# Oneaccount1/recommend-sys

Measured on NVIDIA B200. Metric: similarity_pairs_per_sec, higher is better.
Workload: dtype f64

## Files before the change

recommend-sys_b200/csrc/sim_stream.cu:

```cuda
#include <cstdlib>
#include <cstring>

#include "common.cuh"
#include "sim_terms.cuh"

namespace {

constexpr int SW = RS_STREAM_WARPS;

struct StreamArgs {
    const int64_t *l_ptr;
    const int32_t *l_col;
    const double *l_val;
    const int64_t *l2r;
    const int64_t *r_ptr;
    const int32_t *r_col;
    const double *r_dev;
    const int32_t *row_order;
    const int32_t *cp;
    int32_t n_chunks;
    const double *pmeans;
    const double *left_bias, *right_bias;
    double global_bias, shrinkage;
    double *sims;
    int64_t ld_s;
    int32_t n_left;
    int64_t row_begin, row_end;
    int64_t n_rows;
    int cyc_R;
    int symmetric;
    const int32_t *rank;
    const int32_t *lab_row;
    int32_t n_pop;
    unsigned long long *counter;
};

constexpr int G = 8;


struct PopArgs {
    const int32_t *rows;
    int64_t n_rows;
    const int32_t *rank;
    int32_t n_pop;
    const int32_t *pop_items;
    int32_t n_blk, ld;
    const void *dense;
    int64_t n_first;
    int32_t skip;
};

__device__ __forceinline__ void pop_cp_async16(void *dst, const void *src) {
    asm volatile("cp.async.cg.shared.global [%0], [%1], 16;" ::"r"((uint32_t)__cvta_generic_to_shared(dst)), "l"(src) : "memory");
}
__device__ __forceinline__ void pop_commit() { asm volatile("cp.async.commit_group;" ::: "memory"); }
template <int N> __device__ __forceinline__ void pop_wait() { asm volatile("cp.async.wait_group %0;" ::"n"(N) : "memory"); }

template <int SIM, bool SHRINK, typename DT>
__device__ __forceinline__ void pop_item(const StreamArgs &a, const PopArgs &pa, int64_t item, double *scratch, int lane) {
    constexpr bool U8 = sizeof(DT) == 1;
    double2 *s_a = reinterpret_cast<double2 *>(scratch);
    double *s_rbias = scratch + 64;
    int32_t *s_c = reinterpret_cast<int32_t *>(scratch + 96);
    uint8_t *s_d = reinterpret_cast<uint8_t *>(scratch + 112);
    const DT *__restrict__ dense = static_cast<const DT *>(pa.dense);
    const double nan_v = __longlong_as_double(0x7ff8000000000001ll);
    const int32_t i = pa.rows[item / pa.n_blk];
    const int b = (int)(item % pa.n_blk);
    const int pi = pa.rank[i] < pa.n_pop ? pa.rank[i] : -1;
    if (pi >= 0 && 32 * b > pi) return;
    const int col = 32 * b + lane;
    const int32_t hcol = pa.pop_items[col];
    const bool want = hcol >= 0 && (pi < 0 || col < pi);
    double bh = 0.0;
    if (want && SIM == RS_SIM_PEARSON) bh = a.pmeans[hcol];
    if (want && SIM == RS_SIM_PEARSON_BASELINE) bh = a.global_bias + a.left_bias[hcol];
    double ai = 0.0;
    if (SIM == RS_SIM_PEARSON) ai = a.pmeans[i];
    if (SIM == RS_SIM_PEARSON_BASELINE) ai = a.global_bias + a.left_bias[i];
    double acc0 = 0.0, acc1 = 0.0, acc2 = 0.0, acc3 = 0.0;
    const int64_t eb = a.l_ptr[i], ee = a.l_ptr[i + 1];

    auto apply = [&](bool rated, double rb, const double2 aa, double rbias_u) {
        (void)rbias_u;
        if (SIM == RS_SIM_MSD) {
            const double dd = aa.x - rb;
            const double t = dd * dd;
            if (rated) { acc0 += t; acc1 += 1.0; }
        } else {
            const double t1 = rb * rb, t2 = aa.x * rb;
            if (rated) {
                acc0 += aa.y;
                acc1 += t1;
                acc2 += t2;
                if (SHRINK) acc3 += 1.0;
            }
        }
    };

    if (__any_sync(0xffffffffu, want)) {
        int32_t c_0 = 0, c_1 = 0;
        double v_0 = 0.0, v_1 = 0.0;
        if (eb + lane < ee) { c_0 = a.l_col[eb + lane]; v_0 = a.l_val[eb + lane]; }
        if (eb + 32 + lane < ee) { c_1 = a.l_col[eb + 32 + lane]; v_1 = a.l_val[eb + 32 + lane]; }
        auto issue = [&](int32_t c_l, int64_t x0, int buf) {
            if constexpr (U8) {
#pragma unroll
                for (int h2 = 0; h2 < 2; h2++) {
                    const int p = lane + 32 * h2, u = p >> 1;
                    const int32_t c_u = __shfl_sync(0xffffffffu, c_l, u);
                    if (x0 + u < ee)
                        pop_cp_async16(s_d + buf * 1024 + 32 * u + 16 * (p & 1),
                                       reinterpret_cast<const uint8_t *>(dense) + (int64_t)c_u * pa.ld + 32 * b + 16 * (p & 1));
                }
            }
            pop_commit();
        };
        __syncwarp();
        issue(c_0, eb, 0);
        int buf = 0;
        for (int64_t x0 = eb; x0 < ee; x0 += 32, buf ^= 1) {
            const int32_t c = c_0;
            const double v = v_0;
            c_0 = c_1; v_0 = v_1;
            c_1 = 0; v_1 = 0.0;
            if (x0 + 64 + lane < ee) { c_1 = a.l_col[x0 + 64 + lane]; v_1 = a.l_val[x0 + 64 + lane]; }
            double ra = 0.0, rbias = 0.0;
            if (x0 + lane < ee) {
                if (SIM == RS_SIM_PEARSON) ra = v - ai;
                else if (SIM == RS_SIM_PEARSON_BASELINE) { rbias = a.right_bias[c]; const double bb = ai + rbias; ra = v - bb; }
                else ra = v;
            }
            s_a[lane] = make_double2(ra, ra * ra);
            if (SIM == RS_SIM_PEARSON_BASELINE) s_rbias[lane] = rbias;
            if (!U8) s_c[lane] = c;
            issue(c_0, x0 + 32, buf ^ 1);
            pop_wait<1>();
            __syncwarp();
            const int lim = (ee - x0) < 32 ? (int)(ee - x0) : 32;
            if constexpr (U8) {
                const uint8_t *sd = s_d + buf * 1024 + lane;
#pragma unroll 8
                for (int u = 0; u < lim; u++) {
                    const int code = want ? (int)sd[32 * u] : 0;
                    const double y = __hiloint2double(0x43380000, code) - (6755399441055744.0 + (double)RS_INT8_BIAS);
                    const double2 aa = s_a[u];
                    double rb;
                    double rbias_u = 0.0;
                    if (SIM == RS_SIM_PEARSON) rb = y - bh;
                    else if (SIM == RS_SIM_PEARSON_BASELINE) { rbias_u = s_rbias[u]; const double bb = bh + rbias_u; rb = y - bb; }
                    else rb = y;
                    apply(code != 0, rb, aa, rbias_u);
                }
            } else {
                constexpr int PU = 8;
                for (int u0 = 0; u0 < lim; u0 += PU) {
                    double d[PU];
#pragma unroll
                    for (int g = 0; g < PU; g++) {
                        d[g] = nan_v;
                        if (want && u0 + g < lim) d[g] = dense[(int64_t)s_c[u0 + g] * pa.ld + col];
                    }
#pragma unroll
                    for (int g = 0; g < PU; g++) {
                        const int u = (u0 + g) & 31;
                        apply(d[g] == d[g], d[g], s_a[u], 0.0);
                    }
                }
            }
            __syncwarp();
        }
        pop_wait<0>();
    }

    if (hcol >= 0) {
        double *out = a.sims + (a.cyc_R > 1 ? rs_cyc_local(i, a.cyc_R) : (int64_t)(i - a.row_begin)) * a.ld_s;
        if (pi >= 0 && col == pi) {
            out[hcol] = nan_v;
        } else if (want) {
            const double acc_r[4] = {acc0, acc1, acc2, acc3};
            out[hcol] = sim_value<SIM, SHRINK>(acc_r, 1, a.shrinkage);
        }
    }
}

template <int SIM, bool SHRINK, int SYM, int JC, int POP>
__global__ void __launch_bounds__(SW * 32, 4) sim_stream_kernel(StreamArgs a, PopArgs pa) {
    constexpr int NACC = SHRINK ? 4 : 3;
    extern __shared__ double s_acc_all[];
    const int warp = threadIdx.x >> 5, lane = threadIdx.x & 31;
    double *acc = s_acc_all + (size_t)warp * NACC * JC;
    double *s_ra = s_acc_all + (size_t)SW * NACC * JC + warp * 32;
    const int64_t Q = a.n_chunks;
    const int64_t n_items = a.n_rows * Q;
    const double nan_v = __longlong_as_double(0x7ff8000000000001ll);
    const int32_t *__restrict__ r_col = a.r_col;
    const double *__restrict__ r_dev = a.r_dev;

    for (;;) {
        unsigned long long item = 0;
        if (lane == 0) item = atomicAdd(a.counter, 1ull);
        item = __shfl_sync(0xffffffffu, item, 0);
        if (POP) {
            int64_t d = (int64_t)item;
            if (d >= pa.n_first) d = d >= pa.n_first + n_items ? d - n_items : -1;
            if (d >= pa.n_rows * pa.n_blk) break;
            if (pa.skip && ((d >= 0 && d < pa.n_first && (pa.skip & 1)) || (d < 0 && (pa.skip & 2)) || (d >= pa.n_first && (pa.skip & 4)))) continue;
            if (d >= 0) {
                __syncwarp();
                if (POP == 1) pop_item<SIM, SHRINK, uint8_t>(a, pa, d, acc, lane);
                else pop_item<SIM, SHRINK, double>(a, pa, d, acc, lane);
                __syncwarp();
                continue;
            }
            item -= (unsigned long long)pa.n_first;
        } else if ((int64_t)item >= n_items) break;
        const int64_t q = (int64_t)item % Q;
        const int32_t i = a.row_order[(int64_t)item / Q];
        const int32_t li = POP ? a.rank[i] - a.n_pop : i;
        const int j0 = (int)(q * JC);
        if (SYM == 1 && j0 + JC <= li) continue;
        if (SYM == 2 && j0 > li) continue;

        for (int x = lane; x < NACC * JC; x += 32) acc[x] = 0.0;

        double ai = 0.0;
        if (SIM == RS_SIM_PEARSON) ai = a.pmeans[i];
        if (SIM == RS_SIM_PEARSON_BASELINE) ai = a.global_bias + a.left_bias[i];

        const int64_t eb = a.l_ptr[i], ee = a.l_ptr[i + 1];
        for (int64_t x0 = eb; x0 < ee; x0 += 32) {
            const int64_t e = x0 + lane;
            double ra = 0.0;
            uint32_t lo = 0, self = 0xffffffffu;
            int n = 0;
            if (e < ee) {
                const int32_t c = a.l_col[e];
                const double v = a.l_val[e];
                if (SIM == RS_SIM_PEARSON) ra = v - ai;
                else if (SIM == RS_SIM_PEARSON_BASELINE) { const double bb = ai + a.right_bias[c]; ra = v - bb; }
                else ra = v;
                const int64_t rp = a.r_ptr[c];
                const int32_t *cpc = a.cp + (int64_t)c * (Q + 1) + q;
                int64_t lo64 = rp + cpc[0];
                int64_t hi = rp + cpc[1];
                const int64_t self64 = a.l2r[e];
                if (SYM == 1) { if (self64 + 1 > lo64) lo64 = self64 + 1; }
                else if (SYM == 2) { if (self64 < hi) hi = self64; }
                else self = (uint32_t)self64;
                n = hi > lo64 ? (int)(hi - lo64) : 0;
                lo = (uint32_t)lo64;
            }
            __syncwarp();
            s_ra[lane] = ra;
            __syncwarp();
            const int lim = (ee - x0) < 32 ? (int)(ee - x0) : 32;
            for (int u0 = 0; u0 < lim; u0 += G) {
                int jj[G], nn[G];
                double rbv[G];
#pragma unroll
                for (int g = 0; g < G; g++) {
                    const int u = u0 + g;
                    nn[g] = __shfl_sync(0xffffffffu, n, u);
                    const uint32_t lo_u = __shfl_sync(0xffffffffu, lo, u);
                    uint32_t self_u = 0xffffffffu;
                    if (!SYM) self_u = __shfl_sync(0xffffffffu, self, u);
                    jj[g] = -1;
                    rbv[g] = 0.0;
                    if (lane < nn[g]) {
                        const uint32_t idx = lo_u + (uint32_t)lane;
                        if (SYM || idx != self_u) {
                            jj[g] = r_col[idx] - j0;
                            rbv[g] = r_dev[idx];
                        }
                    }
                }
#pragma unroll
                for (int g = 0; g < G; g++) {
                    if (nn[g] == 0) continue;
                    const double ra_u = s_ra[u0 + g];
                    const double raa_u = ra_u * ra_u;
                    if (jj[g] >= 0) stream_update<SIM, SHRINK, JC>(acc, jj[g], ra_u, raa_u, rbv[g]);
                    if (nn[g] > 32) {
                        const uint32_t lo_u = __shfl_sync(0xffffffffu, lo, u0 + g);
                        uint32_t self_u = 0xffffffffu;
                        if (!SYM) self_u = __shfl_sync(0xffffffffu, self, u0 + g);
                        for (int t = lane + 32; t < nn[g]; t += 32) {
                            const uint32_t idx = lo_u + (uint32_t)t;
                            if (!SYM && idx == self_u) continue;
                            stream_update<SIM, SHRINK, JC>(acc, r_col[idx] - j0, ra_u, raa_u, r_dev[idx]);
                        }
                    }
                    __syncwarp();
                }
            }
        }
        __syncwarp();

        double *out = a.sims + (a.cyc_R > 1 ? rs_cyc_local(i, a.cyc_R) : (int64_t)(i - a.row_begin)) * a.ld_s + (POP ? 0 : j0);
        auto emit = [&](int j, int64_t col) {
            double s = sim_value<SIM, SHRINK>(acc + j, JC, a.shrinkage);
            if (col == (int64_t)li) s = nan_v;
            out[POP ? a.lab_row[col] : j] = s;
        };
        if (POP) {
            for (int j = lane; j < JC; j += 32) {
                const int64_t col = (int64_t)j0 + j;
                if (col >= a.n_left - a.n_pop) break;
                if (SYM == 1 && col < li) continue;
                if (SYM == 2 && col > li) break;
                emit(j, col);
            }
        } else {
            int j_end = a.n_left - j0;
            if (SYM == 2 && li - j0 + 1 < j_end) j_end = li - j0 + 1;
            if (j_end > JC) j_end = JC;
            const int j_beg = SYM == 1 && li > j0 ? li - j0 : 0;
            for (int j = j_beg + lane; j < j_end; j += 32) emit(j, j0 + j);
        }
        __syncwarp();
    }
}



constexpr int HV_CONS = 4, HV_PROD = 8, HV_WARPS = HV_CONS + HV_PROD;
constexpr int HV_SLOTS = 32;
constexpr int HV_DEPTH = 3;
constexpr int HV_JC = 256;

struct HeavyArgs {
    const int32_t *rows;
    int32_t n_rows;
    unsigned long long *counter;
};

__device__ __forceinline__ uint32_t hv_smem_u32(const void *p) { return (uint32_t)__cvta_generic_to_shared(p); }
__device__ __forceinline__ void hv_cp_async4(void *dst, const void *src) {
    asm volatile("cp.async.ca.shared.global [%0], [%1], 4;" ::"r"(hv_smem_u32(dst)), "l"(src) : "memory");
}
__device__ __forceinline__ void hv_cp_async8(void *dst, const void *src) {
    asm volatile("cp.async.ca.shared.global [%0], [%1], 8;" ::"r"(hv_smem_u32(dst)), "l"(src) : "memory");
}
__device__ __forceinline__ void hv_commit() { asm volatile("cp.async.commit_group;" ::: "memory"); }
template <int N> __device__ __forceinline__ void hv_wait() { asm volatile("cp.async.wait_group %0;" ::"n"(N) : "memory"); }

template <int SIM, bool SHRINK>
__global__ void __launch_bounds__(HV_WARPS * 32, 1) sim_stream_heavy_kernel(StreamArgs a, HeavyArgs hv) {
    constexpr int NACC = SHRINK ? 4 : 3;
    extern __shared__ double hv_smem[];
    double *acc = hv_smem;
    double *s_rb = acc + NACC * HV_JC;
    int32_t *s_jc = reinterpret_cast<int32_t *>(s_rb + HV_SLOTS * HV_JC);
    double *s_ra = reinterpret_cast<double *>(s_jc + HV_SLOTS * HV_JC);
    int32_t *s_n = reinterpret_cast<int32_t *>(s_ra + HV_SLOTS);
    volatile int32_t *s_ready = s_n + HV_SLOTS;
    volatile int32_t *s_consumed = s_ready + HV_SLOTS;
    volatile long long *s_item = reinterpret_cast<volatile long long *>(s_consumed + HV_CONS);
    const int warp = threadIdx.x >> 5, lane = threadIdx.x & 31;
    const int64_t Q = a.n_chunks;
    const int64_t n_items = (int64_t)hv.n_rows * Q;
    const double nan_v = __longlong_as_double(0x7ff8000000000001ll);

    for (;;) {
        __syncthreads();
        if (threadIdx.x == 0) *s_item = (long long)atomicAdd(hv.counter, 1ull);
        if (threadIdx.x < HV_SLOTS) s_ready[threadIdx.x] = 0;
        if (threadIdx.x < HV_CONS) s_consumed[threadIdx.x] = 0;
        __syncthreads();
        const int64_t item = *s_item;
        if (item >= n_items) break;
        const int64_t q = item % Q;
        const int32_t i = hv.rows[item / Q];
        const int j0 = (int)(q * HV_JC);
        if (a.symmetric == 1 && j0 + HV_JC <= i) continue;
        if (a.symmetric == 2 && j0 > i) continue;
        const bool diag_chunk = (i >= j0 && i < j0 + HV_JC);
        const int64_t eb = a.l_ptr[i], ee = a.l_ptr[i + 1];
        const int n_ent = (int)(ee - eb);

        if (warp < HV_CONS) {
            const int cw = warp;
#pragma unroll
            for (int z = 0; z < NACC; z++)
                for (int x = lane; x < 64; x += 32) acc[z * HV_JC + 64 * cw + x] = 0.0;
            __syncwarp();
            for (int e = 0; e < n_ent; e++) {
                const int slot = e % HV_SLOTS;
                int word;
                while (((word = s_ready[slot]) >> 9) != e + 1) {}
                __syncwarp();
                const int n = word & 511;
                if (n > 0) {
                    const double ra = s_ra[slot];
                    const double raa = ra * ra;
                    const double *rbs = s_rb + slot * HV_JC;
                    const int32_t *jcs = s_jc + slot * HV_JC;
                    auto apply = [&](int j, double rb) {
                        if (SIM == RS_SIM_MSD) {
                            const double d = ra - rb;
                            acc[j] += d * d;
                            acc[HV_JC + j] += 1.0;
                        } else {
                            acc[j] += raa;
                            acc[HV_JC + j] += rb * rb;
                            acc[2 * HV_JC + j] += ra * rb;
                            if (SHRINK) acc[3 * HV_JC + j] += 1.0;
                        }
                    };
                    if (n <= 64) {
                        int jv[2];
                        double rbv[2];
#pragma unroll
                        for (int u = 0; u < 2; u++) {
                            const int t = lane + 32 * u;
                            jv[u] = t < n ? jcs[t] - j0 : -1;
                            rbv[u] = t < n ? rbs[t] : 0.0;
                        }
#pragma unroll
                        for (int u = 0; u < 2; u++) if (jv[u] >= 0 && (jv[u] >> 6) == cw) apply(jv[u], rbv[u]);
                    } else {
                        int jv[8];
                        double rbv[8];
#pragma unroll
                        for (int u = 0; u < 8; u++) {
                            const int t = lane + 32 * u;
                            jv[u] = t < n ? jcs[t] - j0 : -1;
                            rbv[u] = t < n ? rbs[t] : 0.0;
                        }
#pragma unroll
                        for (int u = 0; u < 8; u++) {
                            const bool mine = jv[u] >= 0 && (jv[u] >> 6) == cw;
                            if (!__any_sync(0xffffffffu, mine)) continue;
                            if (mine) apply(jv[u], rbv[u]);
                        }
                    }
                }
                __syncwarp();
                if (lane == 0) s_consumed[cw] = e + 1;
            }
            __syncwarp();
            double *out = a.sims + (a.cyc_R > 1 ? rs_cyc_local(i, a.cyc_R) : (int64_t)(i - a.row_begin)) * a.ld_s + j0;
            for (int j = 64 * cw + lane; j < 64 * cw + 64; j += 32) {
                const int64_t col = (int64_t)j0 + j;
                if (col >= a.n_left) break;
                if (a.symmetric == 1 && col < i) continue;
                if (a.symmetric == 2 && col > i) break;
                double s = sim_value<SIM, SHRINK>(acc + j, HV_JC, a.shrinkage);
                if (col == (int64_t)i) s = nan_v;
                out[j] = s;
            }
        } else {
            const int p = warp - HV_CONS;
            double ai = 0.0;
            if (SIM == RS_SIM_PEARSON) ai = a.pmeans[i];
            if (SIM == RS_SIM_PEARSON_BASELINE) ai = a.global_bias + a.left_bias[i];
            auto ent_of = [&](int k) { return p + k * HV_PROD; };
            int issued = 0, published = 0;
            auto publish = [&](int k) {
                __syncwarp();
                __threadfence_block();
                if (lane == 0) { const int e = ent_of(k); s_ready[e % HV_SLOTS] = ((e + 1) << 9) | s_n[e % HV_SLOTS]; }
            };
            const int my_total = n_ent > p ? (n_ent - p + HV_PROD - 1) / HV_PROD : 0;
            for (int k0 = 0; k0 < my_total; k0 += 32) {
                const int k_l = k0 + lane;
                double ra_l = 0.0;
                uint32_t lo_l = 0;
                int n_l = 0;
                if (k_l < my_total) {
                    const int64_t e = eb + ent_of(k_l);
                    const int32_t c = a.l_col[e];
                    const double v = a.l_val[e];
                    if (SIM == RS_SIM_PEARSON) ra_l = v - ai;
                    else if (SIM == RS_SIM_PEARSON_BASELINE) { const double bb = ai + a.right_bias[c]; ra_l = v - bb; }
                    else ra_l = v;
                    const int64_t rp = a.r_ptr[c];
                    const int32_t *cpc = a.cp + (int64_t)c * (Q + 1) + q;
                    int64_t lo64 = rp + cpc[0];
                    int64_t hi = rp + cpc[1];
                    if (diag_chunk) {
                        const int64_t self64 = a.l2r[e];
                        if (a.symmetric == 1) { if (self64 + 1 > lo64) lo64 = self64 + 1; }
                        else { if (self64 < hi) hi = self64; }
                    }
                    n_l = hi > lo64 ? (int)(hi - lo64) : 0;
                    lo_l = (uint32_t)lo64;
                }
                const int lim = my_total - k0 < 32 ? my_total - k0 : 32;
                for (int u = 0; u < lim; u++) {
                    const int k = k0 + u;
                    const int e = ent_of(k);
                    const int slot = e % HV_SLOTS;
                    const double ra_u = __shfl_sync(0xffffffffu, ra_l, u);
                    const uint32_t lo_u = __shfl_sync(0xffffffffu, lo_l, u);
                    const int n_u = __shfl_sync(0xffffffffu, n_l, u);
                    for (bool first = true;; first = false) {
                        int done = s_consumed[0];
#pragma unroll
                        for (int z = 1; z < HV_CONS; z++) { const int d = s_consumed[z]; done = d < done ? d : done; }
                        if (done >= e - HV_SLOTS + 1) break;
                        if (first) {
                            hv_wait<0>();
                            while (published < issued) { publish(published); published++; }
                        }
                        __nanosleep(40);
                    }
                    __syncwarp();
                    for (int t = lane; t < n_u; t += 32) {
                        hv_cp_async4(s_jc + slot * HV_JC + t, a.r_col + lo_u + t);
                        hv_cp_async8(s_rb + slot * HV_JC + t, a.r_dev + lo_u + t);
                    }
                    if (lane == 0) { s_ra[slot] = ra_u; s_n[slot] = n_u; }
                    hv_commit();
                    issued++;
                    if (issued - published > HV_DEPTH) {
                        hv_wait<HV_DEPTH>();
                        publish(published);
                        published++;
                    }
                }
            }
            hv_wait<0>();
            while (published < issued) { publish(published); published++; }
        }
    }
}

__device__ __forceinline__ bool pop_owns(int32_t rr, int32_t rc, int32_t n_pop, int lower) {
    if (!lower && rr >= n_pop && rc >= n_pop) return rr < rc;
    return rr > rc;
}

__global__ void symmetrize_kernel(double *__restrict__ s, int64_t ld, int32_t n, int lower) {
    __shared__ double tile[32][33];
    int64_t bi = blockIdx.y, bj = blockIdx.x;
    if (bj > bi) return;
    if (lower) { const int64_t t = bi; bi = bj; bj = t; }
    const int64_t r0 = bi * 32, c0 = bj * 32;
    for (int y = threadIdx.y; y < 32; y += blockDim.y) {
        int64_t sr = c0 + y, sc = r0 + threadIdx.x;
        tile[y][threadIdx.x] = (sr < n && sc < n) ? s[sr * ld + sc] : 0.0;
    }
    __syncthreads();
    for (int y = threadIdx.y; y < 32; y += blockDim.y) {
        int64_t r = r0 + y, c = c0 + threadIdx.x;
        if (r < n && c < n && (lower ? c > r : c < r)) s[r * ld + c] = tile[threadIdx.x][y];
    }
}

struct MirrorArgs {
    double *self;
    const double *peer[RS_MAX_PEERS];
    int64_t ld;
    int32_t n;
    int32_t count, index, lower;
};
__global__ void mirror_kernel(MirrorArgs a) {
    __shared__ double tile[32][33];
    const int64_t bI = blockIdx.y;
    const int64_t gI = bI * a.count + a.index, gJ = blockIdx.x;
    if (a.lower ? gJ < gI : gJ > gI) return;
    const double *src = a.peer[gJ % a.count];
    const int64_t sJ = (gJ / a.count) * RS_CYC_B;
    for (int y = threadIdx.y; y < 32; y += blockDim.y) {
        const int64_t sr = gJ * 32 + y, sc = gI * 32 + threadIdx.x;
        tile[y][threadIdx.x] = (sr < a.n && sc < a.n) ? src[(sJ + y) * a.ld + sc] : 0.0;
    }
    __syncthreads();
    for (int y = threadIdx.y; y < 32; y += blockDim.y) {
        const int64_t r = gI * 32 + y, c = gJ * 32 + threadIdx.x;
        if (r < a.n && c < a.n && (a.lower ? c > r : c < r)) a.self[(bI * 32 + y) * a.ld + c] = tile[threadIdx.x][y];
    }
}

__global__ void symmetrize_pop_kernel(double *__restrict__ s, int64_t ld, int32_t n, int lower,
                                      const int32_t *__restrict__ rank, int32_t n_pop) {
    __shared__ double ta[32][33], tb[32][33];
    __shared__ int32_t rk_a[32], rk_b[32];
    const int64_t bi = blockIdx.y, bj = blockIdx.x;
    if (bj > bi) return;
    const int64_t r0 = bi * 32, c0 = bj * 32;
    if (threadIdx.y == 0) {
        rk_a[threadIdx.x] = r0 + threadIdx.x < n ? rank[r0 + threadIdx.x] : 0;
        rk_b[threadIdx.x] = c0 + threadIdx.x < n ? rank[c0 + threadIdx.x] : 0;
    }
    for (int y = threadIdx.y; y < 32; y += blockDim.y) {
        const int64_t ar = r0 + y, ac = c0 + threadIdx.x, br = c0 + y, bc = r0 + threadIdx.x;
        ta[y][threadIdx.x] = (ar < n && ac < n) ? s[ar * ld + ac] : 0.0;
        tb[y][threadIdx.x] = (br < n && bc < n) ? s[br * ld + bc] : 0.0;
    }
    __syncthreads();
    for (int y = threadIdx.y; y < 32; y += blockDim.y) {
        int64_t r = r0 + y, c = c0 + threadIdx.x;
        if (r < n && c < n && r != c && !pop_owns(rk_a[y], rk_b[threadIdx.x], n_pop, lower)) s[r * ld + c] = tb[threadIdx.x][y];
        if (bi == bj) continue;
        r = c0 + y; c = r0 + threadIdx.x;
        if (r < n && c < n && !pop_owns(rk_b[y], rk_a[threadIdx.x], n_pop, lower)) s[r * ld + c] = ta[threadIdx.x][y];
    }
}

__global__ void mirror_pop_kernel(MirrorArgs a, const int32_t *__restrict__ rank, int32_t n_pop) {
    __shared__ double tile[32][33];
    const int64_t bI = blockIdx.y;
    const int64_t gI = bI * a.count + a.index, gJ = blockIdx.x;
    bool need[4];
    bool any = false;
#pragma unroll
    for (int k = 0; k < 4; k++) {
        const int y = threadIdx.y + 8 * k;
        const int64_t r = gI * 32 + y, c = gJ * 32 + threadIdx.x;
        need[k] = r < a.n && c < a.n && r != c && !pop_owns(rank[r], rank[c], n_pop, a.lower);
        any = any || need[k];
    }
    if (!__syncthreads_or(any)) return;
    const double *src = a.peer[gJ % a.count];
    const int64_t sJ = (gJ / a.count) * RS_CYC_B;
    for (int y = threadIdx.y; y < 32; y += blockDim.y) {
        const int64_t sr = gJ * 32 + y, sc = gI * 32 + threadIdx.x;
        tile[y][threadIdx.x] = (sr < a.n && sc < a.n) ? src[(sJ + y) * a.ld + sc] : 0.0;
    }
    __syncthreads();
#pragma unroll
    for (int k = 0; k < 4; k++) {
        const int y = threadIdx.y + 8 * k;
        if (need[k]) a.self[(bI * 32 + y) * a.ld + gJ * 32 + threadIdx.x] = tile[threadIdx.x][y];
    }
}

}

template <int SIM, bool SHRINK, int SYM, int JC, int POP>
static int32_t launch_stream_pop(rs_knn *h, const StreamArgs &s, const PopArgs &pa, int grid) {
    const int smem = SW * ((SHRINK ? 4 : 3) * JC + 32) * (int)sizeof(double);
    auto kern = sim_stream_kernel<SIM, SHRINK, SYM, JC, POP>;
    RS_CUDA(cudaFuncSetAttribute(kern, cudaFuncAttributeMaxDynamicSharedMemorySize, smem));
    kern<<<grid, SW * 32, smem, h->stream>>>(s, pa);
    return RS_OK;
}
template <int SIM, bool SHRINK, int SYM, int JC>
static int32_t launch_stream_jc(rs_knn *h, const StreamArgs &s, const PopArgs &pa, int grid) {
    if (SYM != 0 && s.rank) {
        if (h->pop_u8) return launch_stream_pop<SIM, SHRINK, SYM ? SYM : 1, JC, 1>(h, s, pa, grid);
        return launch_stream_pop<SIM, SHRINK, SYM ? SYM : 1, JC, 2>(h, s, pa, grid);
    }
    return launch_stream_pop<SIM, SHRINK, SYM, JC, 0>(h, s, pa, grid);
}
template <int SIM, bool SHRINK, int SYM>
static int32_t launch_stream_sym(rs_knn *h, const StreamArgs &s, const PopArgs &pa, int grid) {
    if (h->stream_jc == 128) return launch_stream_jc<SIM, SHRINK, SYM, 128>(h, s, pa, grid);
    return launch_stream_jc<SIM, SHRINK, SYM, 256>(h, s, pa, grid);
}
template <int SIM, bool SHRINK>
static int32_t launch_stream(rs_knn *h, const StreamArgs &s, const PopArgs &pa, int grid) {
    if (h->nnz >= (int64_t)0xffffffffll) {
        rs_set_error("stream path indexes the ratings with 32 bits (nnz=%lld)", (long long)h->nnz);
        return RS_ERR_UNSUPPORTED;
    }
    if (s.symmetric == 2) return launch_stream_sym<SIM, SHRINK, 2>(h, s, pa, grid);
    return s.symmetric ? launch_stream_sym<SIM, SHRINK, 1>(h, s, pa, grid) : launch_stream_sym<SIM, SHRINK, 0>(h, s, pa, grid);
}

template <int SIM, bool SHRINK>
static int32_t launch_heavy(rs_knn *h, const StreamArgs &a, const HeavyArgs &hv) {
    constexpr int NACC = SHRINK ? 4 : 3;
    const int smem = (NACC * HV_JC + HV_SLOTS * HV_JC) * 8 + HV_SLOTS * HV_JC * 4 + HV_SLOTS * 8 + HV_SLOTS * 4 * 2 + HV_CONS * 4 + 64;
    auto kern = sim_stream_heavy_kernel<SIM, SHRINK>;
    RS_CUDA(cudaFuncSetAttribute(kern, cudaFuncAttributeMaxDynamicSharedMemorySize, smem));
    int sms = 148;
    cudaDeviceGetAttribute(&sms, cudaDevAttrMultiProcessorCount, h->device);
    int64_t grid = (int64_t)hv.n_rows * a.n_chunks;
    if (grid > sms) grid = sms;
    kern<<<(unsigned)grid, HV_WARPS * 32, smem, h->aux_stream>>>(a, hv);
    h->prof.total_launches += 1;
    return RS_OK;
}

static int32_t rs_heavy_rows_launch(rs_knn *h, const StreamArgs &a, const HeavyArgs &hv) {
    switch (h->p.sim) {
    case RS_SIM_COSINE: return launch_heavy<RS_SIM_COSINE, false>(h, a, hv);
    case RS_SIM_MSD: return launch_heavy<RS_SIM_MSD, false>(h, a, hv);
    case RS_SIM_PEARSON: return launch_heavy<RS_SIM_PEARSON, false>(h, a, hv);
    case RS_SIM_PEARSON_BASELINE:
        return h->p.shrinkage > 0.0 ? launch_heavy<RS_SIM_PEARSON_BASELINE, true>(h, a, hv)
                                    : launch_heavy<RS_SIM_PEARSON_BASELINE, false>(h, a, hv);
    default: rs_set_error("unknown similarity %d", h->p.sim); return RS_ERR_INVALID;
    }
}

int32_t rs_sim_stream_launch(rs_knn *h) {
    StreamArgs a{};
    a.l_ptr = h->l_ptr; a.l_col = h->l_col; a.l_val = h->l_val; a.l2r = h->l2r;
    a.r_ptr = h->r_ptr; a.r_col = h->r_col; a.r_dev = h->r_dev; a.cp = h->cp; a.n_chunks = h->n_chunks;
    const bool cyc = h->cyc_R > 1;
    a.row_order = h->n_work_rows >= 0 ? h->row_order : h->row_order + h->row_begin;
    a.n_rows = h->n_work_rows >= 0 ? h->n_work_rows : h->row_end - h->row_begin;
    a.cyc_R = h->cyc_R;
    a.pmeans = h->pmeans; a.left_bias = h->left_bias; a.right_bias = h->right_bias;
    a.global_bias = h->global_bias; a.shrinkage = h->p.shrinkage;
    a.sims = h->sims; a.ld_s = h->ld_s; a.n_left = h->n_left;
    a.row_begin = h->row_begin; a.row_end = h->row_end;
    a.symmetric = h->force_sym ? 1 : ((h->row_begin == 0 && h->row_end == h->n_left) || cyc) ? (h->stream_lower ? 2 : 1) : 0;
    a.counter = reinterpret_cast<unsigned long long *>(h->d_flags + 2);
    RS_CUDA(cudaMemsetAsync(a.counter, 0, 8, h->stream));
    const bool pop = h->n_pop > 0;
    PopArgs pa{};
    if (pop) {
        if (a.symmetric == 0 || h->force_sym) {
            rs_set_error("popular columns were split off, but this Fit does not compute a triangle of the full matrix");
            return RS_ERR_INVALID;
        }
        a.r_ptr = h->w_ptr; a.r_col = h->w_col; a.r_dev = h->w_dev;
        a.rank = h->rank; a.lab_row = h->lab_row; a.n_pop = h->n_pop;
        pa.rows = h->row_all; pa.n_rows = h->n_all_rows;
        pa.rank = h->rank; pa.n_pop = h->n_pop; pa.pop_items = h->pop_items;
        pa.n_blk = h->pop_ld / 32; pa.ld = h->pop_ld;
        pa.dense = h->pop_dense;
        pa.n_first = (h->n_all_rows - a.n_rows) * pa.n_blk;
        if (const char *e = getenv("RS_KNN_STREAM_SKIP")) pa.skip = atoi(e);
    }
    const bool heavy = !pop && h->n_heavy > 0 && a.symmetric != 0 && !h->force_sym && h->stream_jc == HV_JC;
    if (heavy) {
        HeavyArgs hv{};
        hv.rows = h->row_heavy; hv.n_rows = h->n_heavy;
        hv.counter = reinterpret_cast<unsigned long long *>(h->d_flags + 12);
        RS_CUDA(cudaMemsetAsync(hv.counter, 0, 8, h->stream));
        RS_CUDA(cudaEventRecord(h->ev_fork, h->stream));
        RS_CUDA(cudaStreamWaitEvent(h->aux_stream, h->ev_fork, 0));
        RS_TRY(rs_heavy_rows_launch(h, a, hv));
        RS_CUDA(cudaEventRecord(h->ev_join, h->aux_stream));
    }
    if (a.n_rows <= 0 && !(pop && pa.n_rows > 0)) {
        if (heavy) RS_CUDA(cudaStreamWaitEvent(h->stream, h->ev_join, 0));
        return RS_OK;
    }
    int sms = 148;
    cudaDeviceGetAttribute(&sms, cudaDevAttrMultiProcessorCount, h->device);
    const int64_t items = a.n_rows * (int64_t)h->n_chunks + (pop ? pa.n_rows * pa.n_blk : 0);
    int64_t grid = (int64_t)sms * 4;
    if (grid > (items + SW - 1) / SW) grid = (items + SW - 1) / SW;
    switch (h->p.sim) {
    case RS_SIM_COSINE: RS_TRY((launch_stream<RS_SIM_COSINE, false>(h, a, pa, (int)grid))); break;
    case RS_SIM_MSD: RS_TRY((launch_stream<RS_SIM_MSD, false>(h, a, pa, (int)grid))); break;
    case RS_SIM_PEARSON: RS_TRY((launch_stream<RS_SIM_PEARSON, false>(h, a, pa, (int)grid))); break;
    case RS_SIM_PEARSON_BASELINE:
        if (h->p.shrinkage > 0.0) RS_TRY((launch_stream<RS_SIM_PEARSON_BASELINE, true>(h, a, pa, (int)grid)));
        else RS_TRY((launch_stream<RS_SIM_PEARSON_BASELINE, false>(h, a, pa, (int)grid)));
        break;
    default: rs_set_error("unknown similarity %d", h->p.sim); return RS_ERR_INVALID;
    }
    if (heavy) RS_CUDA(cudaStreamWaitEvent(h->stream, h->ev_join, 0));
    h->prof.sim_launches++;
    h->prof.total_launches++;
    RS_CUDA(cudaGetLastError());
    return RS_OK;
}

int32_t rs_mirror_launch(rs_knn *h) {
    MirrorArgs a{};
    a.self = h->sims;
    for (int q = 0; q < h->cyc_R; q++) a.peer[q] = h->peer_sims[q];
    a.peer[h->cyc_r] = h->sims;
    a.ld = h->ld_s; a.n = h->n_left; a.count = h->cyc_R; a.index = h->cyc_r; a.lower = h->stream_lower ? 1 : 0;
    const int64_t nblk = ((int64_t)h->n_left + RS_CYC_B - 1) / RS_CYC_B;
    const int64_t own = (nblk - h->cyc_r + h->cyc_R - 1) / h->cyc_R;
    if (own <= 0) return RS_OK;
    dim3 grid((unsigned)nblk, (unsigned)own), block(32, 8);
    if (h->n_pop > 0) mirror_pop_kernel<<<grid, block, 0, h->stream>>>(a, h->rank, h->n_pop);
    else mirror_kernel<<<grid, block, 0, h->stream>>>(a);
    h->prof.total_launches++;
    RS_CUDA(cudaGetLastError());
    return RS_OK;
}

int32_t rs_symmetrize_launch(rs_knn *h) {
    if (h->cyc_R > 1) return RS_OK;
    if (!(h->row_begin == 0 && h->row_end == h->n_left)) return RS_OK;
    const unsigned t = (unsigned)((h->n_left + 31) / 32);
    dim3 grid(t, t), block(32, 8);
    if (h->n_pop > 0) symmetrize_pop_kernel<<<grid, block, 0, h->stream>>>(h->sims, h->ld_s, h->n_left, h->stream_lower ? 1 : 0, h->rank, h->n_pop);
    else symmetrize_kernel<<<grid, block, 0, h->stream>>>(h->sims, h->ld_s, h->n_left, h->stream_lower ? 1 : 0);
    h->prof.total_launches++;
    RS_CUDA(cudaGetLastError());
    return RS_OK;
}
```

Baseline: 6.585 billion.

## Load-balance POP streaming via warp prefix-sum flattening and prefetched neighbor lookups

For the POP kernel path, each 32-edge chunk's per-edge neighbor ranges are flattened into one contiguous work list using a warp prefix scan. Lanes then find their owning edge by binary search over shuffles, so every lane gets work even when per-edge neighbor counts are short or uneven. The l_col/l_val loads and r_ptr/cp/l2r lookups for the next chunk are software-prefetched one iteration ahead. Because lanes in a batch can now update the same accumulator column, conflicts are serialized with match_any rounds. This adds scan, search and conflict-handling overhead and registers in exchange for less idle lane time.

```diff
diff --git a/recommend-sys_b200/csrc/sim_stream.cu b/recommend-sys_b200/csrc/sim_stream.cu
--- a/recommend-sys_b200/csrc/sim_stream.cu
+++ b/recommend-sys_b200/csrc/sim_stream.cu
@@ -36,6 +36,7 @@
 };
 
 constexpr int G = 8;
+constexpr int W = 4;
 
 
 struct PopArgs {
@@ -229,69 +230,163 @@
         if (SIM == RS_SIM_PEARSON_BASELINE) ai = a.global_bias + a.left_bias[i];
 
         const int64_t eb = a.l_ptr[i], ee = a.l_ptr[i + 1];
-        for (int64_t x0 = eb; x0 < ee; x0 += 32) {
-            const int64_t e = x0 + lane;
-            double ra = 0.0;
-            uint32_t lo = 0, self = 0xffffffffu;
-            int n = 0;
-            if (e < ee) {
-                const int32_t c = a.l_col[e];
-                const double v = a.l_val[e];
-                if (SIM == RS_SIM_PEARSON) ra = v - ai;
-                else if (SIM == RS_SIM_PEARSON_BASELINE) { const double bb = ai + a.right_bias[c]; ra = v - bb; }
-                else ra = v;
-                const int64_t rp = a.r_ptr[c];
-                const int32_t *cpc = a.cp + (int64_t)c * (Q + 1) + q;
-                int64_t lo64 = rp + cpc[0];
-                int64_t hi = rp + cpc[1];
-                const int64_t self64 = a.l2r[e];
-                if (SYM == 1) { if (self64 + 1 > lo64) lo64 = self64 + 1; }
-                else if (SYM == 2) { if (self64 < hi) hi = self64; }
-                else self = (uint32_t)self64;
-                n = hi > lo64 ? (int)(hi - lo64) : 0;
-                lo = (uint32_t)lo64;
-            }
-            __syncwarp();
-            s_ra[lane] = ra;
-            __syncwarp();
-            const int lim = (ee - x0) < 32 ? (int)(ee - x0) : 32;
-            for (int u0 = 0; u0 < lim; u0 += G) {
-                int jj[G], nn[G];
-                double rbv[G];
-#pragma unroll
-                for (int g = 0; g < G; g++) {
-                    const int u = u0 + g;
-                    nn[g] = __shfl_sync(0xffffffffu, n, u);
-                    const uint32_t lo_u = __shfl_sync(0xffffffffu, lo, u);
-                    uint32_t self_u = 0xffffffffu;
-                    if (!SYM) self_u = __shfl_sync(0xffffffffu, self, u);
-                    jj[g] = -1;
-                    rbv[g] = 0.0;
-                    if (lane < nn[g]) {
-                        const uint32_t idx = lo_u + (uint32_t)lane;
-                        if (SYM || idx != self_u) {
-                            jj[g] = r_col[idx] - j0;
-                            rbv[g] = r_dev[idx];
+        if constexpr (POP == 0) {
+            for (int64_t x0 = eb; x0 < ee; x0 += 32) {
+                const int64_t e = x0 + lane;
+                double ra = 0.0;
+                uint32_t lo = 0, self = 0xffffffffu;
+                int n = 0;
+                if (e < ee) {
+                    const int32_t c = a.l_col[e];
+                    const double v = a.l_val[e];
+                    if (SIM == RS_SIM_PEARSON) ra = v - ai;
+                    else if (SIM == RS_SIM_PEARSON_BASELINE) { const double bb = ai + a.right_bias[c]; ra = v - bb; }
+                    else ra = v;
+                    const int64_t rp = a.r_ptr[c];
+                    const int32_t *cpc = a.cp + (int64_t)c * (Q + 1) + q;
+                    int64_t lo64 = rp + cpc[0];
+                    int64_t hi = rp + cpc[1];
+                    const int64_t self64 = a.l2r[e];
+                    if (SYM == 1) { if (self64 + 1 > lo64) lo64 = self64 + 1; }
+                    else if (SYM == 2) { if (self64 < hi) hi = self64; }
+                    else self = (uint32_t)self64;
+                    n = hi > lo64 ? (int)(hi - lo64) : 0;
+                    lo = (uint32_t)lo64;
+                }
+                __syncwarp();
+                s_ra[lane] = ra;
+                __syncwarp();
+                const int lim = (ee - x0) < 32 ? (int)(ee - x0) : 32;
+                for (int u0 = 0; u0 < lim; u0 += G) {
+                    int jj[G], nn[G];
+                    double rbv[G];
+#pragma unroll
+                    for (int g = 0; g < G; g++) {
+                        const int u = u0 + g;
+                        nn[g] = __shfl_sync(0xffffffffu, n, u);
+                        const uint32_t lo_u = __shfl_sync(0xffffffffu, lo, u);
+                        uint32_t self_u = 0xffffffffu;
+                        if (!SYM) self_u = __shfl_sync(0xffffffffu, self, u);
+                        jj[g] = -1;
+                        rbv[g] = 0.0;
+                        if (lane < nn[g]) {
+                            const uint32_t idx = lo_u + (uint32_t)lane;
+                            if (SYM || idx != self_u) {
+                                jj[g] = r_col[idx] - j0;
+                                rbv[g] = r_dev[idx];
+                            }
                         }
                     }
-                }
-#pragma unroll
-                for (int g = 0; g < G; g++) {
-                    if (nn[g] == 0) continue;
-                    const double ra_u = s_ra[u0 + g];
-                    const double raa_u = ra_u * ra_u;
-                    if (jj[g] >= 0) stream_update<SIM, SHRINK, JC>(acc, jj[g], ra_u, raa_u, rbv[g]);
-                    if (nn[g] > 32) {
-                        const uint32_t lo_u = __shfl_sync(0xffffffffu, lo, u0 + g);
+#pragma unroll
+                    for (int g = 0; g < G; g++) {
+                        if (nn[g] == 0) continue;
+                        const double ra_u = s_ra[u0 + g];
+                        const double raa_u = ra_u * ra_u;
+                        if (jj[g] >= 0) stream_update<SIM, SHRINK, JC>(acc, jj[g], ra_u, raa_u, rbv[g]);
+                        if (nn[g] > 32) {
+                            const uint32_t lo_u = __shfl_sync(0xffffffffu, lo, u0 + g);
+                            uint32_t self_u = 0xffffffffu;
+                            if (!SYM) self_u = __shfl_sync(0xffffffffu, self, u0 + g);
+                            for (int t = lane + 32; t < nn[g]; t += 32) {
+                                const uint32_t idx = lo_u + (uint32_t)t;
+                                if (!SYM && idx == self_u) continue;
+                                stream_update<SIM, SHRINK, JC>(acc, r_col[idx] - j0, ra_u, raa_u, r_dev[idx]);
+                            }
+                        }
+                        __syncwarp();
+                    }
+                }
+            }
+        } else {
+            int32_t c_nx = 0;
+            double v_nx = 0.0;
+            uint32_t rp_k = 0, p0_k = 0, p1_k = 0, s_k = 0;
+            double v_k = 0.0, rbias_k = 0.0;
+            auto lookup = [&](int64_t e, int32_t c, double v) {
+                rp_k = p0_k = p1_k = s_k = 0;
+                v_k = v;
+                if (e < ee) {
+                    rp_k = (uint32_t)a.r_ptr[c];
+                    const int32_t *cpc = a.cp + (int64_t)c * (Q + 1) + q;
+                    p0_k = (uint32_t)cpc[0];
+                    p1_k = (uint32_t)cpc[1];
+                    s_k = (uint32_t)a.l2r[e];
+                    if (SIM == RS_SIM_PEARSON_BASELINE) rbias_k = a.right_bias[c];
+                }
+            };
+            if (eb + lane < ee) { c_nx = a.l_col[eb + lane]; v_nx = a.l_val[eb + lane]; }
+            lookup(eb + lane, c_nx, v_nx);
+            c_nx = 0; v_nx = 0.0;
+            if (eb + 32 + lane < ee) { c_nx = a.l_col[eb + 32 + lane]; v_nx = a.l_val[eb + 32 + lane]; }
+            for (int64_t x0 = eb; x0 < ee; x0 += 32) {
+                double ra;
+                if (SIM == RS_SIM_PEARSON) ra = v_k - ai;
+                else if (SIM == RS_SIM_PEARSON_BASELINE) { const double bb = ai + rbias_k; ra = v_k - bb; }
+                else ra = v_k;
+                if (x0 + lane >= ee) ra = 0.0;
+                uint32_t lo = rp_k + p0_k, hi = rp_k + p1_k, self = 0xffffffffu;
+                if (SYM == 1) { if (s_k + 1 > lo) lo = s_k + 1; }
+                else if (SYM == 2) { if (s_k < hi) hi = s_k; }
+                else self = s_k;
+                const int n = hi > lo ? (int)(hi - lo) : 0;
+                lookup(x0 + 32 + lane, c_nx, v_nx);
+                c_nx = 0; v_nx = 0.0;
+                if (x0 + 64 + lane < ee) { c_nx = a.l_col[x0 + 64 + lane]; v_nx = a.l_val[x0 + 64 + lane]; }
+                int end = n;
+#pragma unroll
+                for (int d = 1; d < 32; d <<= 1) {
+                    const int t = __shfl_up_sync(0xffffffffu, end, d);
+                    if (lane >= d) end += t;
+                }
+                const int T = __shfl_sync(0xffffffffu, end, 31);
+                const uint32_t off = lo - (uint32_t)(end - n);
+                __syncwarp();
+                s_ra[lane] = ra;
+                __syncwarp();
+                for (int base = 0; base < T; base += 32 * W) {
+                    int jw[W], uw[W];
+                    double rbw[W];
+#pragma unroll
+                    for (int w = 0; w < W; w++) {
+                        jw[w] = -1 - lane;
+                        rbw[w] = 0.0;
+                        uw[w] = 0;
+                        const int p = base + 32 * w + lane;
+                        if (base + 32 * w >= T) continue;
+                        int u = 0;
+#pragma unroll
+                        for (int s = 16; s >= 1; s >>= 1)
+                            if (__shfl_sync(0xffffffffu, end, u + s - 1) <= p) u += s;
+                        const uint32_t idx = __shfl_sync(0xffffffffu, off, u) + (uint32_t)p;
                         uint32_t self_u = 0xffffffffu;
-                        if (!SYM) self_u = __shfl_sync(0xffffffffu, self, u0 + g);
-                        for (int t = lane + 32; t < nn[g]; t += 32) {
-                            const uint32_t idx = lo_u + (uint32_t)t;
-                            if (!SYM && idx == self_u) continue;
-                            stream_update<SIM, SHRINK, JC>(acc, r_col[idx] - j0, ra_u, raa_u, r_dev[idx]);
+                        if (!SYM) self_u = __shfl_sync(0xffffffffu, self, u);
+                        uw[w] = u;
+                        if (p < T && (SYM || idx != self_u)) {
+                            jw[w] = r_col[idx] - j0;
+                            rbw[w] = r_dev[idx];
                         }
                     }
-                    __syncwarp();
+#pragma unroll
+                    for (int w = 0; w < W; w++) {
+                        const int wb = base + 32 * w;
+                        if (wb >= T) break;
+                        const double ra_u = s_ra[uw[w]];
+                        const double raa_u = ra_u * ra_u;
+                        const bool act = jw[w] >= 0;
+                        const int last = T - wb < 32 ? T - wb - 1 : 31;
+                        if (__shfl_sync(0xffffffffu, uw[w], 0) == __shfl_sync(0xffffffffu, uw[w], last)) {
+                            if (act) stream_update<SIM, SHRINK, JC>(acc, jw[w], ra_u, raa_u, rbw[w]);
+                        } else {
+                            const unsigned m = __match_any_sync(0xffffffffu, jw[w]);
+                            const int rank = __popc(m & ((1u << lane) - 1u));
+                            const int rounds = (int)__reduce_max_sync(0xffffffffu, (unsigned)rank) + 1;
+                            for (int r = 0; r < rounds; r++) {
+                                if (r) __syncwarp();
+                                if (act && rank == r) stream_update<SIM, SHRINK, JC>(acc, jw[w], ra_u, raa_u, rbw[w]);
+                            }
+                        }
+                        __syncwarp();
+                    }
                 }
             }
         }
```

After: 6.672 billion (median of 6 runs). 1.3% higher.
